# d3sm0/gym_pomdp

Hardware: AMD Instinct MI355X
Metric: env steps/sec (whole node), RockSample(7,8) batch=2^20, 1/2/4/8 MI355X (higher is better)
Workload: dtype int32

## Files before the change

### gym_pomdp_amd/csrc/episodes.hip

```cpp
#include "kernels_common.hip.h"
#include <cstring>

namespace pomdp {

template <class Env>
__global__ __launch_bounds__(BLOCK) void reset_where_kernel(const typename Env::Params p, uint32_t *__restrict__ state,
                                                            int32_t *__restrict__ ob, uint8_t *__restrict__ done,
                                                            const uint8_t *__restrict__ where, int64_t n, RngKey key, uint32_t lane0)
{
    __shared__ typename Env::Shared sh;
    Env::stage(sh, p, (int)threadIdx.x);
    __syncthreads();
    const int64_t i = (int64_t)blockIdx.x * BLOCK + threadIdx.x;
    if (i >= n) return;
    const bool fresh = !where || where[i] != 0;
    int o = -1;
    if (fresh) {
        typename Env::State st;
        o = Env::reset(sh, p, st, key, lane0 + (uint32_t)i);
        Env::store(st, state, n, (uint32_t)i, true);
        if (done) done[i] = 0;
    }
    if (ob) ob[i] = o;
}
// ... 153 lines not shown
        if constexpr (TAPE) a_tape = col.nxt;
    }
    if (in_range) {
        Env::store(st, state_w, n, rel, false);
        done[wg0 + rel] = frozen ? 1 : 0;
        if constexpr (RETS) out.finish(0, rel);
    }
    if (TAPE && n_bad && tape.err) atomicAdd(tape.err, n_bad);
}

template <class Env, class L, class Pol>
__global__ __launch_bounds__(BLOCK) void episodes_quad_kernel(uint32_t *__restrict__ state, uint8_t *__restrict__ done,
                                                              void *__restrict__ out0, void *__restrict__ out1, uint64_t discount_bits,
                                                              int64_t n, RngKey key0, uint32_t lane0, int k_steps, int64_t rec,
                                                              const typename Env::Params p, TapeRef tape)
{
    constexpr bool RETS = L::ID == LAYOUT_RETURNS;
    constexpr int W = Env::WORDS;
    using S = typename Env::S;
    __shared__ typename Env::Shared sh;
    __shared__ typename Env::RecTab tab;
    const uint32_t n_act = (uint32_t)Env::n_actions(p);
    const uint32_t l0 = blockIdx.x * (uint32_t)(4 * BLOCK) + 4u * threadIdx.x, glane0 = lane0 + l0;
    Pol pol(tape, l0, glane0, key0, key0, n_act, k_steps);
    using Out = typename std::conditional<RETS, EpisodeReturns<Env, 4>, QuadOut<L>>::type;
    Out out = [&]() {
        if constexpr (RETS) return Out(reinterpret_cast<double *>(out0), reinterpret_cast<uint32_t *>(out1), bits_f64(discount_bits), rec);
        else return Out(out0, nullptr, nullptr, nullptr, rec, l0);
    }();
    typename Env::State st[4];
    bool frozen[4];
    uint32_t a_cur[4] = {0, 0, 0, 0};
    {
        const u32x4 lo = ld_stream4(state + l0);
        u32x4 hi = {0, 0, 0, 0};
        if (W == 2) hi = ld_stream4(state + n + l0);
        const uint32_t dn = ld_stream(reinterpret_cast<const uint32_t *>(done + l0));
        if constexpr (Pol::TAPE) {
            const u32x4 f = pol.first();
#pragma unroll
            for (int j = 0; j < 4; ++j) a_cur[j] = f[j];
        }
#pragma unroll
        for (int j = 0; j < 4; ++j) {
            st[j].s = (S)((uint64_t)lo[j] | ((uint64_t)hi[j] << 32));
            frozen[j] = ((dn >> (8 * j)) & 0xFFu) != 0u;
        }
// ... 197 lines not shown
```

### gym_pomdp_amd/csrc/fused_impl.hip.h

```cpp
#pragma once
#include "kernels_common.hip.h"

namespace pomdp {

template <class L, class Pol, int LPT = 4, bool SROW = false>
struct FusedCtx {
    uint32_t l0, glane0;
    uint64_t t0;
    typename lanes_out<L, LPT, SROW>::type out;
    typename lanes_policy<Pol, LPT>::type pol;
    uint32_t n_bad;
    __device__ __forceinline__ FusedCtx(int32_t *action, int32_t *ob, void *reward, uint8_t *done, int64_t rec, uint32_t lane0,
                                        const RngKey &key0, const RngKey &akey0, uint32_t n_act, int k_steps, const TapeRef &tape)
        : l0(blockIdx.x * (uint32_t)(LPT * BLOCK) + (uint32_t)LPT * threadIdx.x), glane0(lane0 + l0),
          t0(((uint64_t)key0.t_hi << 32) | key0.t_lo), out(action, ob, reward, done, rec, l0),
          pol(tape, l0, glane0, key0, akey0, n_act, k_steps), n_bad(0) {}
    __device__ __forceinline__ void first(int gen_first, int (&a_cur)[LPT])
    {
        if constexpr (LPT == 4) {
            const u32x4 a4 = out.first(pol, gen_first);
#pragma unroll
            for (int j = 0; j < 4; ++j) a_cur[j] = (int)a4[j];
        } else {
            uint32_t a2[LPT];
            pol.first(a2);
#pragma unroll
            for (int j = 0; j < LPT; ++j) a_cur[j] = (int)a2[j];
        }
    }
    __device__ __forceinline__ RngKey key(const RngKey &key0, int s) const
    {
        RngKey k = key0;
        k.t_lo = (uint32_t)(t0 + (uint64_t)s); k.t_hi = (uint32_t)((t0 + (uint64_t)s) >> 32);
        return k;
    }
    __device__ __forceinline__ void advance(int s, uint32_t (&a_next)[LPT], int (&a_cur)[LPT])
    {
        pol.end(s, a_next);
#pragma unroll
        for (int j = 0; j < LPT; ++j) a_cur[j] = (int)a_next[j];
    }
    __device__ __forceinline__ void finish(int k_steps)
    {
        pol.count_bad(n_bad);
        out.finish(k_steps);
    }
};
#define POMDP_FUSED_STEP_LOOP(prio_, s_)                                                                              \
    wait_loads();                                                                                                      \
    _Pragma("unroll 1") for (int seg_ = 0, s_ = 0; seg_ < 4; ++seg_)                                                   \
        for (const int seg_end_ = (prio_).segment(seg_); s_ < seg_end_; ++s_)


template <class Env, int LPT, bool SIMPLE, bool TAB = false, class L = Columns, bool TAPE = false>
__global__ __launch_bounds__(BLOCK) void steps_kernel(uint32_t *__restrict__ state, int32_t *__restrict__ action,
                                                      int32_t *__restrict__ ob, typename Env::Reward *__restrict__ reward,
                                                      uint8_t *__restrict__ done, uint32_t *__restrict__ err, int64_t n,
                                                      RngKey key0, uint32_t lane0, int flags, RngKey akey0, int k_steps,
                                                      int64_t rec, const typename Env::Params p, TapeRef tape)
{
    static_assert(!TAPE || LPT == 1, "a tape drives the one-lane-per-thread instantiations");
    __shared__ typename Env::Shared sh;
    constexpr bool REC = TAB;
    __shared__ typename step_tab_of<Env, TAB>::type tab;
    static_assert(!TAB || (SIMPLE && LPT == 1), "the table-driven step serves the SIMPLE one-lane-per-thread instantiation");
    const bool auto_reset = SIMPLE || (flags & POMDP_AUTO_RESET);
    const uint32_t wg0 = blockIdx.x * (uint32_t)(BLOCK * LPT);
    const uint32_t last = SIMPLE ? (uint32_t)(BLOCK * LPT - 1) : (uint32_t)((uint64_t)(n - 1) - wg0);
    LaneOut<L, typename Env::Reward, LPT> out(action, ob, reward, done, rec, wg0);
    uint32_t *const state_w = state + wg0;
    constexpr bool COLS = L::ID == POMDP_LAYOUT_COLUMNS;
    uint32_t rel[LPT], glane[LPT];
    bool in_range[LPT], was_done[LPT], ever_fresh[LPT];
    int a_cur[LPT];
// ... 197 lines not shown
        for (int seg = 0, s = 0; seg < 4; ++seg)
        for (const int seg_end = prio.segment(seg); s < seg_end; ++s) step_body(s, s & 3);
    }
#pragma unroll
    for (int j = 0; j < LPT; ++j)
        if (in_range[j]) { Env::store(st[j], state_w, n, rel[j], ever_fresh[j]); out.finish(j, rel[j], k_steps); }
}

template <class Env, class L, class Pol, int LPT, class Form>
__device__ __forceinline__ void steps_quad_body(uint32_t *__restrict__ state, int32_t *__restrict__ action,
                                                int32_t *__restrict__ ob, int32_t *__restrict__ reward,
                                                uint8_t *__restrict__ done, int64_t n, RngKey key0, uint32_t lane0,
                                                RngKey akey0, int k_steps, int64_t rec, int gen_first,
                                                const typename Env::Params &p, TapeRef tape)
{
    static_assert(LPT == 4 || LPT == 2, "a quad or half a quad per thread");
    constexpr int W = Env::WORDS;
    using S = typename Env::S;
    __shared__ typename Env::Shared sh;
    __shared__ typename Form::Tab tab;
    const uint32_t n_act = (uint32_t)Env::n_actions(p);
    constexpr bool AHEAD2 = Pol::TAPE && LPT == 4;
    using PolT = typename std::conditional<AHEAD2, TapeQuadAhead, Pol>::type;
    FusedCtx<L, PolT, LPT, true> cx(action, ob, reward, done, rec, lane0, key0, akey0, n_act, k_steps, tape);
    const uint32_t l0 = cx.l0, glane0 = cx.glane0;
    const uint32_t e0 = LPT == 4 ? 0u : (glane0 & 2u);
    typename Env::State st[LPT];
    int a_cur[LPT];
    uint32_t sp0 = 0, sp1 = 0, gp0 = 0, gp1 = 0;
    {
        uint32_t s_lo[LPT], s_hi[LPT];
        if constexpr (LPT == 4) {
            const u32x4 lo = ld_stream4(state + l0);
            u32x4 hi = {0, 0, 0, 0};
            if (W == 2) hi = ld_stream4(state + n + l0);
#pragma unroll
            for (int j = 0; j < 4; ++j) { s_lo[j] = lo[j]; s_hi[j] = hi[j]; }
        } else {
            const u32x2 lo = ld_stream2(state + l0);
            u32x2 hi = {0, 0};
            if (W == 2) hi = ld_stream2(state + n + l0);
#pragma unroll
            for (int j = 0; j < 2; ++j) { s_lo[j] = lo[j]; s_hi[j] = hi[j]; }
        }
        cx.first(gen_first, a_cur);
#pragma unroll
        for (int j = 0; j < LPT; ++j) {
            if constexpr (W == 1) st[j].s = Form::from_mem(s_lo[j]);
            else st[j].s = (S)((uint64_t)s_lo[j] | ((uint64_t)s_hi[j] << 32));
        }
    }
    Env::stage(sh, p, (int)threadIdx.x);
    __syncthreads();
    if constexpr (W == 1) { if (Form::builds(threadIdx.x)) Form::build(tab, sh, p, (int)threadIdx.x); }
    else Env::build_rec_tab(tab, sh, p, (int)threadIdx.x);
    __syncthreads();
    const int K = p.num_rocks;
    const uint32_t start = (uint32_t)p.start_x | ((uint32_t)p.start_y << 4);
    uint32_t start_rot = start, tie_bound = 0;
    if constexpr (W == 1) { start_rot = Form::start_word(start); asm volatile("" : "+v"(start_rot)); }
    const LoopPrio prio(k_steps);
    constexpr uint32_t SENSOR_BLOCK = Env::SENSOR_BLOCK;
    const PhiloxFixed sensor_fx = philox_fixed(glane0 >> 2, ((uint32_t)POMDP_STREAM_STEP << 24) | SENSOR_BLOCK, key0.k1);
    const PhiloxFixed gate_fx = philox_fixed(glane0 >> 2, (uint32_t)POMDP_STREAM_STEP << 24, key0.k1);
    if constexpr (W == 1) tie_bound = Form::tie_bound(K);
    auto step_body = [&](const int s, const auto par_) __attribute__((always_inline)) {
        constexpr int PAR = decltype(par_)::value;
        const RngKey key = cx.key(key0, s);
        uint32_t H[LPT], G[LPT];
        if constexpr (LPT == 4) {
            const uint4 sw = philox4x32_10_fixed(sensor_fx, key.t_lo, key.t_hi, key.k0, key.k1);
            H[0] = sw.x; H[1] = sw.y; H[2] = sw.z; H[3] = sw.w;
        } else {
            pair_shared(s, e0 != 0u, [&](int sb) { return Env::quad_block(cx.key(key0, sb), glane0, SENSOR_BLOCK); }, H, sp0, sp1);
        }
        uint32_t a_next[LPT];
        if constexpr (AHEAD2) cx.pol.template begin_par<PAR>(s, a_next);
        else cx.pol.begin(s, a_next);
        bool acts[LPT];
#pragma unroll
        for (int j = 0; j < LPT; ++j) acts[j] = true;
        if constexpr (Env::STOCHASTIC) {
            if constexpr (LPT == 4) {
                const uint4 gw = philox4x32_10_fixed(gate_fx, key.t_lo, key.t_hi, key.k0, key.k1);
                G[0] = gw.x; G[1] = gw.y; G[2] = gw.z; G[3] = gw.w;
            } else {
                pair_shared(s, e0 != 0u, [&](int sb) { return Env::quad_block(cx.key(key0, sb), glane0, 0u); }, G, gp0, gp1);
            }
#pragma unroll
            for (int j = 0; j < LPT; ++j)
                acts[j] = Env::k53_le(G[j], (uint32_t)(p.act_thr >> 26), (uint32_t)p.act_thr & Env::LO_MASK,
                                      [&]() { return Env::elem(Env::quad_block(key, glane0, 1u), e0 + (uint32_t)j); }) != (p.act_gt != 0);
        }
        uint32_t rec[LPT], a_taken[LPT];
#pragma unroll
        for (int j = 0; j < LPT; ++j) a_taken[j] = (uint32_t)a_cur[j];
        bool valid[LPT];
#pragma unroll
        for (int j = 0; j < LPT; ++j) valid[j] = !Pol::TAPE || a_taken[j] < n_act;
        auto low_word = [&](int j) __attribute__((always_inline)) {
            return Env::elem(Env::quad_block(rare_key(key), glane0 + (uint32_t)j, SENSOR_BLOCK + 1u), e0 + (uint32_t)j);
        };
        if constexpr (W == 1) {
            uint32_t fresh[LPT], sn[LPT];
            typename Form::Entry ef[LPT];
            Form::template fresh<LPT>(H, key, glane0, K, start_rot, tie_bound, fresh);
#pragma unroll
// ... 43 lines not shown
                              [&]() { return low_word(j); });
                if constexpr (Env::STOCHASTIC) {
                    sj = acts[j] ? sj : st[j].s;
                    rec[j] = acts[j] ? rec[j] : a_taken[j];
                }
                if constexpr (Pol::TAPE) {
                    sj = valid[j] ? sj : st[j].s;
                    rec[j] = valid[j] ? rec[j] : a_taken[j];
                    cx.n_bad += (uint32_t)!valid[j];
                }
                st[j].s = sj;
            }
        }
        cx.out.put_records(rec, a_next);
        if constexpr (AHEAD2) {
            cx.pol.template end_par<PAR>(s, a_next);
#pragma unroll
            for (int j = 0; j < LPT; ++j) a_cur[j] = (int)a_next[j];
        } else cx.advance(s, a_next, a_cur);
    };
    if constexpr (AHEAD2) {
        wait_loads();
        _Pragma("unroll 1") for (int seg = 0, s = 0; seg < 4; ++seg)
            for (const int seg_end = prio.template segment<2>(seg); s < seg_end; s += 2) {
                step_body(s, std::integral_constant<int, 0>{});
                if (s + 1 < seg_end) step_body(s + 1, std::integral_constant<int, 1>{});
            }
    } else {
        POMDP_FUSED_STEP_LOOP(prio, s) step_body(s, std::integral_constant<int, 0>{});
    }
    cx.finish(k_steps);
    uint32_t w_lo[LPT];
#pragma unroll
    for (int j = 0; j < LPT; ++j) {
        w_lo[j] = (uint32_t)st[j].s;
        if constexpr (W == 1) w_lo[j] = Form::to_mem(w_lo[j]);
    }
    if constexpr (LPT == 4) {
        st_stream4(state + l0, w_lo[0], w_lo[1], w_lo[2], w_lo[3]);
        if (W == 2)
            st_stream4(state + n + l0, (uint32_t)((uint64_t)st[0].s >> 32), (uint32_t)((uint64_t)st[1].s >> 32),
                       (uint32_t)((uint64_t)st[2].s >> 32), (uint32_t)((uint64_t)st[3].s >> 32));
    } else {
        st_stream2(state + l0, w_lo[0], w_lo[1]);
        if (W == 2) st_stream2(state + n + l0, (uint32_t)((uint64_t)st[0].s >> 32), (uint32_t)((uint64_t)st[1].s >> 32));
    }
}
template <class Env, class L = Columns, class Pol = SyntheticQuad, int LPT = 4>
__global__ __launch_bounds__(BLOCK) void steps_quad_kernel(uint32_t *__restrict__ state, int32_t *__restrict__ action,
                                                           int32_t *__restrict__ ob, int32_t *__restrict__ reward,
                                                           uint8_t *__restrict__ done, int64_t n, RngKey key0, uint32_t lane0,
                                                           RngKey akey0, int k_steps, int64_t rec, int gen_first,
// ... 5 lines not shown
template <class Env, class L = Columns, class Pol = SyntheticQuad, int LPT = 4>
__global__ __launch_bounds__(BLOCK) void steps_quad_popc_kernel(uint32_t *__restrict__ state, int32_t *__restrict__ action,
                                                                int32_t *__restrict__ ob, int32_t *__restrict__ reward,
                                                                uint8_t *__restrict__ done, int64_t n, RngKey key0, uint32_t lane0,
                                                                RngKey akey0, int k_steps, int64_t rec, int gen_first,
                                                                const typename Env::Params p, TapeRef tape)
{
    static_assert(Env::WORDS == 1, "two state words take steps_quad_kernel");
    steps_quad_body<Env, L, Pol, LPT, typename Env::RecRot>(state, action, ob, reward, done, n, key0, lane0, akey0, k_steps, rec, gen_first, p, tape);
}

template <bool TAB, class L = Columns, class Pol = SyntheticQuad, int LPT = 4>
__global__ __launch_bounds__(BLOCK) void tag_steps_quad_kernel(uint32_t *__restrict__ state, int32_t *__restrict__ action,
                                                               int32_t *__restrict__ ob, float *__restrict__ reward,
                                                               uint8_t *__restrict__ done, int64_t n, RngKey key0,
                                                               uint32_t lane0, RngKey akey0, int k_steps, int64_t rec,
                                                               int gen_first, const TagEnv::Params p, TapeRef tape)
{
    using Env = TagEnv;
    static_assert(LPT == 4 || LPT == 2, "a quad or half a quad per thread");
    __shared__ Env::Shared sh;
    __shared__ typename std::conditional<TAB, Env::StepTab, NoTab>::type tab;
    const uint32_t n_act = (uint32_t)Env::n_actions(p);
    FusedCtx<L, Pol, LPT> cx(action, ob, reward, done, rec, lane0, key0, akey0, n_act, k_steps, tape);
    const uint32_t l0 = cx.l0, glane0 = cx.glane0;
    const uint32_t e0 = LPT == 4 ? 0u : (glane0 & 2u);
    Env::State st[LPT];
    int a_cur[LPT];
    uint32_t sp0 = 0, sp1 = 0;
    {
        if constexpr (LPT == 4) {
            const u32x4 s4 = ld_stream4(state + l0);
            cx.first(gen_first, a_cur);
#pragma unroll
            for (int j = 0; j < 4; ++j) st[j].w = s4[j];
        } else {
            const u32x2 s2 = ld_stream2(state + l0);
            cx.first(gen_first, a_cur);
#pragma unroll
            for (int j = 0; j < 2; ++j) st[j].w = s2[j];
        }
    }
    Env::stage(sh, p, (int)threadIdx.x);
    __syncthreads();
    if constexpr (TAB) {
        Env::build_tab(tab, sh, p, (int)threadIdx.x);
        __syncthreads();
    }
    const LoopPrio prio(k_steps);
    POMDP_FUSED_STEP_LOOP(prio, s) {
        const RngKey key = cx.key(key0, s);
        uint32_t a_next[LPT];
        cx.pol.begin(s, a_next);
        int o[LPT], d[LPT];
        float r[LPT];
        uint32_t a_taken[LPT], W[LPT];
#pragma unroll
        for (int j = 0; j < LPT; ++j) a_taken[j] = (uint32_t)a_cur[j];
        if constexpr (LPT == 4) {
            const uint4 qw = Env::quad_block(key, glane0, 0u);
            W[0] = qw.x; W[1] = qw.y; W[2] = qw.z; W[3] = qw.w;
        } else {
            pair_shared(s, e0 != 0u, [&](int sb) { return Env::quad_block(cx.key(key0, sb), glane0, 0u); }, W, sp0, sp1);
        }
#pragma unroll
        for (int j = 0; j < LPT; ++j) {
            Env::Flight f;
            const bool valid = !Pol::TAPE || a_taken[j] < n_act;
            const Env::State before = st[j];
            const int a = valid ? a_cur[j] : 0;
            if constexpr (TAB) Env::step_one_opponent_tab(tab, st[j], a, o[j], r[j], d[j], f);
            else Env::step_one_opponent_pre(sh, p, st[j], a, o[j], r[j], d[j], f);
            const uint32_t lane = glane0 + (uint32_t)j;
// ... 70 lines not shown
        if (threadIdx.x < 4) {
            const uint32_t f = (T.fail >> 16) - 1u, nb = (T.nb >> 16) - 1u;
            tp[threadIdx.x] = (((threadIdx.x & 1u) ? nb : f) << 16) | ((threadIdx.x & 2u) ? nb : f);
        }
    } else {
#pragma unroll
    for (int kb = 0; kb < NB; ++kb) {
        uint32_t m = 0;
        for (int i = 0; i < p.n_machines; ++i) m |= (((p.nb_mask[i] >> (8 * kb)) & threadIdx.x) != 0u ? 1u : 0u) << i;
        nbf8[kb][threadIdx.x] = m;
    }
    }
    if (threadIdx.x < 3 * 68) {
        const int kind = (int)threadIdx.x / 68, b = (int)threadIdx.x % 68;
        double r = (double)b;
        if (kind == 1) r -= .1;
        if (kind == 2) r -= 2.5;
        rtab[kind][b] = (float)r;
    }
    __syncthreads();
    const uint32_t all_up = p.n_machines >= 32 ? 0xFFFFFFFFu : ((1u << p.n_machines) - 1u);
    const int M2 = 2 * p.n_machines;
    const LoopPrio prio(k_steps);
    POMDP_FUSED_STEP_LOOP(prio, s) {
        const RngKey key = cx.key(key0, s);
        uint32_t a_next[4];
        cx.pol.begin(s, a_next);
        const uint4 q0 = Env::quad_block(key, glane0, 0u), q1 = Env::quad_block(key, glane0, 1u), q2 = Env::quad_block(key, glane0, 2u);
        const uint32_t W0[4] = {q0.x, q0.y, q0.z, q0.w}, W1[4] = {q1.x, q1.y, q1.z, q1.w};
        const uint32_t W2[4] = {q2.x, q2.y, q2.z, q2.w};
        bool valid[4] = {true, true, true, true};
        if constexpr (Pol::TAPE) {
#pragma unroll
            for (int j = 0; j < 4; ++j) { valid[j] = (uint32_t)a_cur[j] < n_act; cx.n_bad += (uint32_t)!valid[j]; }
        }
        const uint32_t a_taken[4] = {(uint32_t)a_cur[0], (uint32_t)a_cur[1], (uint32_t)a_cur[2], (uint32_t)a_cur[3]};
        if constexpr (Pol::TAPE) {
#pragma unroll
            for (int j = 0; j < 4; ++j) a_cur[j] = valid[j] ? a_cur[j] : M2;
        }
        uint32_t kill[4], todo[4], near[4], tie16[4];
        int base[4];
        bool truthful[4], pend[4], need[4];
        bool any_need = false;
#pragma unroll
        for (int j = 0; j < 4; ++j) {
            const uint32_t s0 = st[j] & all_up;
// ... 100 lines not shown
    cx.finish(k_steps);
    st_stream4(state + l0, st[0], st[1], st[2], st[3]);
}

template <class L, int MW, bool VIS_LDS = false> struct quad_waves { static constexpr int value = (L::ID == LAYOUT_RETURNS && MW >= 3 && !VIS_LDS) ? 4 : 1; };
template <int MW, class L = Columns, class Pol = SyntheticQuad, int LPT = 4, bool VIS_LDS = false>
__global__ __launch_bounds__(BLOCK) __attribute__((amdgpu_waves_per_eu(quad_waves<L, MW, VIS_LDS>::value))) void battleship_steps_quad_kernel(uint32_t *__restrict__ state, int32_t *__restrict__ action,
                                                                      int32_t *__restrict__ ob, int32_t *__restrict__ reward,
                                                                      uint8_t *__restrict__ done, int64_t n, RngKey key0,
                                                                      uint32_t lane0, RngKey akey0, int k_steps, int64_t rec,
                                                                      int gen_first, const pomdp_battleship_params p, TapeRef tape)
{
    using Env = BattleShipEnv<MW>;
    using Mask = typename Env::Mask;
    static_assert(LPT == 4 || LPT == 2, "a quad or half a quad per thread");
    constexpr int LOG = LPT == 4 ? 2 : 1;
    __shared__ uint32_t occ_lds[MW][LPT][BLOCK], next_lds[MW][LPT][BLOCK], vis_lds[VIS_LDS ? MW : 1][VIS_LDS ? LPT : 1][VIS_LDS ? BLOCK : 1];
    __shared__ uint8_t task_lds[BLOCK / 64][64 * LPT];
    __shared__ uint8_t ts_lds[BLOCK / 64][64 * LPT];
    __shared__ typename Env::SeqTables seq;
    Env::stage_seq(seq, p, (int)threadIdx.x);
    const int wv = (int)(threadIdx.x >> 6), me = (int)(threadIdx.x & 63u), tid = (int)threadIdx.x;
    const uint32_t n_act = (uint32_t)Env::n_actions(p);
    FusedCtx<L, Pol, LPT> cx(action, ob, reward, done, rec, lane0, key0, akey0, n_act, k_steps, tape);
    const uint32_t l0 = cx.l0, glane0 = cx.glane0, wave0 = glane0 - (uint32_t)LPT * (uint32_t)me;
    int rem[LPT];
    Mask vis[VIS_LDS ? 1 : LPT];
    int a_cur[LPT];
    {
        typename std::conditional<LPT == 4, u32x4, u32x2>::type w[3 * MW];
#pragma unroll
        for (int q = 0; q < 3 * MW; ++q) {
            if constexpr (LPT == 4) w[q] = ld_stream4(state + (int64_t)q * n + l0);
            else w[q] = ld_stream2(state + (int64_t)q * n + l0);
        }
        cx.first(gen_first, a_cur);
#pragma unroll
        for (int j = 0; j < LPT; ++j) {
            rem[j] = (int)(w[2 * MW - 1][j] >> 26);
            if constexpr (!VIS_LDS) vis[j].lo = vis[j].hi = 0;
#pragma unroll
            for (int q = 0; q < MW; ++q) {
                occ_lds[q][j][tid] = w[q][j];
                if constexpr (VIS_LDS) vis_lds[q][j][tid] = q == MW - 1 ? (w[MW + q][j] & 0x03FFFFFFu) : w[MW + q][j];
                else vis[j].set_word(q, w[MW + q][j]);
                next_lds[q][j][tid] = w[2 * MW + q][j];
            }
// ... 31 lines not shown
        bld.idle();
        take(my);
        while (__any(my >= 0)) {
            const uint4 b4 = philox4x32_10(wave0 + (uint32_t)bidx, bt_lo, bt_hi, ((uint32_t)POMDP_STREAM_NEXT << 24) | (blk & 0xFFFFFFu), key0.k0, key0.k1);
            ++blk;
            Env::feed2(bld, seq, bc, b4.x, b4.y);
            Env::feed2(bld, seq, bc, b4.z, b4.w);
            const bool fin = my >= 0 && !bld.busy();
            const uint64_t fm = __ballot(fin);
            if (fm != 0ull) {
                if (fin) {
#pragma unroll
                    for (int w = 0; w < MW; ++w) next_lds[w][bidx & (LPT - 1)][64 * wv + (bidx >> LOG)] = (uint32_t)(bld.occ >> (32 * w));
                }
                const int r = (int)__builtin_amdgcn_mbcnt_hi((uint32_t)(fm >> 32), __builtin_amdgcn_mbcnt_lo((uint32_t)fm, 0u));
                if (fin) { my = next_task + r < ntask ? next_task + r : -1; bld.idle(); take(my); }
                next_task += __popcll(fm);
            }
        }
        __builtin_amdgcn_fence(__ATOMIC_RELEASE, "wavefront");
        __builtin_amdgcn_wave_barrier();
    };
    const LoopPrio prio(k_steps, k_steps >= 32);
    POMDP_FUSED_STEP_LOOP(prio, s) {
        uint32_t a_taken[LPT];
        bool valid[LPT];
#pragma unroll
        for (int j = 0; j < LPT; ++j) { a_taken[j] = (uint32_t)a_cur[j]; valid[j] = true; }
        if constexpr (Pol::TAPE) {
#pragma unroll
            for (int j = 0; j < LPT; ++j) { valid[j] = a_taken[j] < n_act; cx.n_bad += (uint32_t)!valid[j]; a_cur[j] = valid[j] ? a_cur[j] : 0; }
        }
        uint32_t ow[LPT], vw[LPT];
#pragma unroll
        for (int j = 0; j < LPT; ++j) {
            ow[j] = occ_lds[a_cur[j] >> 5][j][tid];
            vw[j] = VIS_LDS ? vis_lds[a_cur[j] >> 5][j][tid] : 0u;
        }
        uint32_t a_next[LPT];
        cx.pol.begin(s, a_next);
        uint32_t o4[LPT], r4[LPT], d4[LPT];
        bool d[LPT], again = false, any_d = false;
#pragma unroll
        for (int j = 0; j < LPT; ++j) {
            const int a = a_cur[j];
            int r;
            uint32_t ob_j;
// ... 78 lines not shown
template <class Env, class L = Columns, class Pol = SyntheticQuad>
__global__ __launch_bounds__(BLOCK) void steps_quad_generic_kernel(uint32_t *__restrict__ state, int32_t *__restrict__ action,
                                                                   int32_t *__restrict__ ob,
                                                                   typename Env::Reward *__restrict__ reward,
                                                                   uint8_t *__restrict__ done, int64_t n, RngKey key0,
                                                                   uint32_t lane0, RngKey akey0, int k_steps, int64_t rec,
                                                                   int gen_first, const typename Env::Params p, TapeRef tape)
{
    static_assert(Env::WORDS == 1 && sizeof(typename Env::Reward) == 4, "one state word, 4-byte rewards");
    __shared__ typename Env::Shared sh;
    const uint32_t n_act = (uint32_t)Env::n_actions(p);
    FusedCtx<L, Pol> cx(action, ob, reward, done, rec, lane0, key0, akey0, n_act, k_steps, tape);
    const uint32_t l0 = cx.l0, glane0 = cx.glane0;
    typename Env::State st[4];
    int a_cur[4];
    {
#pragma unroll
        for (int j = 0; j < 4; ++j) Env::load(st[j], state, n, l0 + (uint32_t)j);
        cx.first(gen_first, a_cur);
    }
    Env::stage(sh, p, (int)threadIdx.x);
    __syncthreads();
    const LoopPrio prio(k_steps);
    POMDP_FUSED_STEP_LOOP(prio, s) {
        const RngKey key = cx.key(key0, s);
        uint32_t a_next[4];
        cx.pol.begin(s, a_next);
        uint32_t o4[4], r4[4], d4[4], rc[4] = {0, 0, 0, 0};
        const uint32_t a_taken[4] = {(uint32_t)a_cur[0], (uint32_t)a_cur[1], (uint32_t)a_cur[2], (uint32_t)a_cur[3]};
        uint32_t W[4] = {0, 0, 0, 0};
        if constexpr (quad_word_env<Env>::value) {
            const uint4 qw = Env::quad_block(key, glane0, 0u);
            W[0] = qw.x; W[1] = qw.y; W[2] = qw.z; W[3] = qw.w;
        }
#pragma unroll
        for (int j = 0; j < 4; ++j) {
            int o, d;
            typename Env::Reward r;
            const uint32_t lane = glane0 + (uint32_t)j;
            const bool valid = !Pol::TAPE || a_taken[j] < n_act;
            const typename Env::State before = st[j];
            const int a = valid ? a_cur[j] : 0;
            if constexpr (quad_word_env<Env>::value)
                Env::step_word(p, st[j], a, W[j], [&]() { return Env::elem(Env::quad_block(key, lane, 1u), (uint32_t)j); }, o, r, d);
            else
                Env::step(sh, p, st[j], a, key, lane, o, r, d);
            if constexpr (Pol::TAPE) { if (!valid) { st[j] = before; o = 0; r = 0; d = 0; cx.n_bad++; } }
// ... 248 lines not shown
```

### gym_pomdp_amd/csrc/philox.hip.h

```cpp
#pragma once
#include <hip/hip_runtime.h>
#include <stdint.h>

namespace pomdp {

template <bool STREAM = true, class T>
__device__ __forceinline__ T ld_stream(const T *p) { return STREAM ? __builtin_nontemporal_load(p) : *p; }
template <bool STREAM = true, class T>
__device__ __forceinline__ void st_stream(T *p, T v)
{
    if (STREAM) __hip_atomic_store(p, v, __ATOMIC_RELAXED, __HIP_MEMORY_SCOPE_AGENT);
    else *p = v;
}

typedef uint32_t u32x4 __attribute__((ext_vector_type(4)));
__device__ __forceinline__ u32x4 ld_stream4(const uint32_t *p) { return __builtin_nontemporal_load(reinterpret_cast<const u32x4 *>(p)); }
__device__ __forceinline__ void st_stream4(uint32_t *p, uint32_t a, uint32_t b, uint32_t c, uint32_t d)
{
    __builtin_nontemporal_store(u32x4{a, b, c, d}, reinterpret_cast<u32x4 *>(p));
}

typedef uint32_t u32x2 __attribute__((ext_vector_type(2)));
__device__ __forceinline__ u32x2 ld_stream2(const uint32_t *p) { return __builtin_nontemporal_load(reinterpret_cast<const u32x2 *>(p)); }
__device__ __forceinline__ void st_stream2(uint32_t *p, uint32_t a, uint32_t b)
// ... 8 lines not shown

__device__ __forceinline__ uint4 philox4x32_10(uint32_t c0, uint32_t c1, uint32_t c2, uint32_t c3,
                                               uint32_t k0, uint32_t k1)
{
#pragma unroll
    for (int r = 0; r < 10; ++r) {
        const uint64_t p0 = (uint64_t)0xD2511F53u * c0;
        const uint64_t p1 = (uint64_t)0xCD9E8D57u * c2;
        const uint32_t n0 = __builtin_amdgcn_bitop3_b32((uint32_t)(p1 >> 32), c1, k0, 0x96);
        const uint32_t n2 = __builtin_amdgcn_bitop3_b32((uint32_t)(p0 >> 32), c3, k1, 0x96);
        c1 = (uint32_t)p1;
        c3 = (uint32_t)p0;
        c0 = n0;
        c2 = n2;
        k0 += 0x9E3779B9u;
        k1 += 0xBB67AE85u;
    }
    return make_uint4(c0, c1, c2, c3);
}

struct PhiloxFixed {
    uint32_t a_lo;
    uint32_t d_hi, d_lo;
};
__device__ __forceinline__ PhiloxFixed philox_fixed(uint32_t c0, uint32_t c3, uint32_t k1)
{
    const uint64_t a = (uint64_t)0xD2511F53u * c0;
    const uint64_t d = (uint64_t)0xCD9E8D57u * ((uint32_t)(a >> 32) ^ c3 ^ k1);
    return PhiloxFixed{(uint32_t)a, (uint32_t)(d >> 32), (uint32_t)d};
}
__device__ __forceinline__ uint4 philox4x32_10_fixed(const PhiloxFixed &f, uint32_t c1, uint32_t c2, uint32_t k0, uint32_t k1)
{
    const uint64_t b = (uint64_t)0xCD9E8D57u * c2;
    const uint32_t u0 = (uint32_t)(b >> 32) ^ c1 ^ k0;
    const uint64_t c = (uint64_t)0xD2511F53u * u0;
    k0 += 0x9E3779B9u; k1 += 0xBB67AE85u;
    uint32_t x0 = f.d_hi ^ ((uint32_t)b ^ k0);
    uint32_t x2 = f.a_lo ^ ((uint32_t)(c >> 32) ^ k1);
    uint32_t x1 = f.d_lo, x3 = (uint32_t)c;
    k0 += 0x9E3779B9u; k1 += 0xBB67AE85u;
    {
        const uint64_t p0 = (uint64_t)0xD2511F53u * x0;
        const uint64_t p1 = (uint64_t)0xCD9E8D57u * x2;
        const uint32_t n0 = __builtin_amdgcn_bitop3_b32((uint32_t)(p1 >> 32), x1, k0, 0x96);
        const uint32_t n2 = (uint32_t)(p0 >> 32) ^ (x3 ^ k1);
        x1 = (uint32_t)p1; x3 = (uint32_t)p0; x0 = n0; x2 = n2;
        k0 += 0x9E3779B9u; k1 += 0xBB67AE85u;
    }
#pragma unroll
    for (int r = 3; r < 10; ++r) {
        const uint64_t p0 = (uint64_t)0xD2511F53u * x0;
        const uint64_t p1 = (uint64_t)0xCD9E8D57u * x2;
        const uint32_t n0 = __builtin_amdgcn_bitop3_b32((uint32_t)(p1 >> 32), x1, k0, 0x96);
        const uint32_t n2 = __builtin_amdgcn_bitop3_b32((uint32_t)(p0 >> 32), x3, k1, 0x96);
        x1 = (uint32_t)p1; x3 = (uint32_t)p0; x0 = n0; x2 = n2;
        k0 += 0x9E3779B9u; k1 += 0xBB67AE85u;
    }
    return make_uint4(x0, x1, x2, x3);
}

__device__ __forceinline__ RngKey rare_key(const RngKey &k)
{
    RngKey r = k;
    asm volatile("" : "+s"(r.t_lo), "+s"(r.t_hi));
    return r;
}

__device__ __forceinline__ uint4 stream_block(const RngKey &k, uint32_t lane, uint32_t stream, uint32_t block)
{
// ... 42 lines not shown
```

### gym_pomdp_amd/csrc/traj_out.hip.h

```cpp
#pragma once
#include "envs.hip.h"

namespace pomdp {

constexpr int LAYOUT_RETURNS = 100;
template <bool ACT> struct ColumnsT { static constexpr int ID = POMDP_LAYOUT_COLUMNS; static constexpr const char *NAME = "Columns"; static constexpr bool CODES = false; };
using Columns = ColumnsT<true>;
using ColumnsNoAct = ColumnsT<false>;
struct Blocked { static constexpr int ID = POMDP_LAYOUT_BLOCKED; static constexpr const char *NAME = "Blocked"; static constexpr bool CODES = false; };
struct Packed  { static constexpr int ID = POMDP_LAYOUT_PACKED;  static constexpr const char *NAME = "Packed";  static constexpr bool CODES = true; };
struct Narrow  { static constexpr int ID = POMDP_LAYOUT_NARROW;  static constexpr const char *NAME = "Narrow";  static constexpr bool CODES = true; };
template <class Env> struct Returns { static constexpr int ID = LAYOUT_RETURNS; static constexpr const char *NAME = "Returns"; static constexpr bool CODES = true; using E = Env; };

constexpr int TRAJ_BLOCK_LANES = 256;
constexpr int TRAJ_BLOCK_BYTES = 13 * TRAJ_BLOCK_LANES;

static __device__ __forceinline__ uint32_t pack_record(uint32_t a, uint32_t o, uint32_t rcode, uint32_t d)
{
    return a | (o << 8) | ((rcode & 0xFFu) << 16) | (d << 24);
}

struct TapeRef {
    const uint8_t *base;
    int64_t stride;
// ... 1 lines not shown
};

template <class T>
struct TapeColumn {
    const uint8_t *p;
    int64_t stride;
    int last;
    T first, nxt;
    __device__ __forceinline__ T row(int r) const
    {
        r = r < last ? r : last;
        return ld_stream(reinterpret_cast<const T *>(p + (int64_t)r * stride));
    }
    __device__ __forceinline__ TapeColumn(const TapeRef &t, uint32_t col, int k_steps)
        : p(t.base + col), stride(t.stride), last(k_steps - 1), nxt(0) { first = row(0); }
    __device__ __forceinline__ void request(int s) { nxt = row(s + 1); }
};
struct NoColumn {
    uint8_t first, nxt;
    __device__ __forceinline__ NoColumn(const TapeRef &, uint32_t, int) : first(0), nxt(0) {}
    __device__ __forceinline__ void request(int) {}
};

struct SyntheticQuad {
    static constexpr bool TAPE = false;
    uint32_t glane0, n_act, k0, k1;
    uint64_t ta0;
    PhiloxFixed fx;
    __device__ __forceinline__ SyntheticQuad(const TapeRef &, uint32_t, uint32_t glane0_, const RngKey &key0, const RngKey &akey0, uint32_t n_act_, int)
        : glane0(glane0_), n_act(n_act_), k0(key0.k0), k1(key0.k1), ta0(((uint64_t)akey0.t_hi << 32) | akey0.t_lo),
          fx(philox_fixed(glane0_ >> 2, (uint32_t)POMDP_STREAM_ACTION << 24, key0.k1)) {}
    __device__ __forceinline__ uint4 block(uint64_t ta) const
    {
        return philox4x32_10_fixed(fx, (uint32_t)ta, (uint32_t)(ta >> 32), k0, k1);
    }
    __device__ __forceinline__ u32x4 first() const
    {
        const uint4 w = block(ta0 - 1ull);
        return u32x4{__umulhi(w.x, n_act), __umulhi(w.y, n_act), __umulhi(w.z, n_act), __umulhi(w.w, n_act)};
    }
    __device__ __forceinline__ void begin(int s, uint32_t (&a)[4]) const
    {
        const uint4 pw = block(ta0 + (uint64_t)s);
        a[0] = __umulhi(pw.x, n_act); a[1] = __umulhi(pw.y, n_act); a[2] = __umulhi(pw.z, n_act); a[3] = __umulhi(pw.w, n_act);
    }
    __device__ __forceinline__ void end(int, uint32_t (&)[4]) const {}
    __device__ __forceinline__ void count_bad(uint32_t) const {}
};
struct TapeQuad {
    static constexpr bool TAPE = true;
    TapeColumn<uint32_t> col;
    uint32_t *err;
    static __device__ __forceinline__ void unpack(uint32_t w, uint32_t (&a)[4])
    {
        a[0] = w & 0xFFu; a[1] = __builtin_amdgcn_ubfe(w, 8u, 8u); a[2] = __builtin_amdgcn_ubfe(w, 16u, 8u); a[3] = w >> 24;
    }
    __device__ __forceinline__ TapeQuad(const TapeRef &t, uint32_t l0, uint32_t, const RngKey &, const RngKey &, uint32_t, int k_steps)
        : col(t, l0, k_steps), err(t.err) {}
    __device__ __forceinline__ u32x4 first() const
    {
        uint32_t a[4];
        unpack(col.first, a);
        return u32x4{a[0], a[1], a[2], a[3]};
    }
    __device__ __forceinline__ void begin(int s, uint32_t (&a)[4]) { col.request(s); a[0] = a[1] = a[2] = a[3] = 0; }
    __device__ __forceinline__ void end(int, uint32_t (&a)[4]) const { unpack(col.nxt, a); }
    __device__ __forceinline__ void count_bad(uint32_t n_bad) const { if (n_bad && err) atomicAdd(err, n_bad); }
};

struct TapeQuadAhead {
    static constexpr bool TAPE = true;
    TapeColumn<uint32_t> col;
    uint32_t *err;
    uint32_t even, odd;
    __device__ __forceinline__ TapeQuadAhead(const TapeRef &t, uint32_t l0, uint32_t, const RngKey &, const RngKey &, uint32_t, int k_steps)
        : col(t, l0, k_steps), err(t.err), even(0), odd(col.row(1)) {}
    __device__ __forceinline__ u32x4 first() const
    {
        uint32_t a[4];
        TapeQuad::unpack(col.first, a);
        return u32x4{a[0], a[1], a[2], a[3]};
    }
    template <int PAR> __device__ __forceinline__ void begin_par(int s, uint32_t (&a)[4])
    {
        if constexpr (PAR == 0) even = col.row(s + 2); else odd = col.row(s + 2);
        a[0] = a[1] = a[2] = a[3] = 0;
    }
    template <int PAR> __device__ __forceinline__ void end_par(int, uint32_t (&a)[4]) const { TapeQuad::unpack(PAR == 0 ? odd : even, a); }
    __device__ __forceinline__ void count_bad(uint32_t n_bad) const { if (n_bad && err) atomicAdd(err, n_bad); }
};

static __device__ __forceinline__ uint32_t pair_swap(uint32_t v)
{
    return (uint32_t)__builtin_amdgcn_update_dpp((int)v, (int)v, 0xB1, 0xF, 0xF, false);
}
template <class BlockOfStep>
static __device__ __forceinline__ void pair_shared(int s, bool hi, BlockOfStep block_of_step, uint32_t (&w)[2], uint32_t &odd0, uint32_t &odd1)
{
    if ((s & 1) == 0) {
        const uint4 b = block_of_step(s + (hi ? 1 : 0));
        const uint32_t r0 = pair_swap(hi ? b.x : b.z), r1 = pair_swap(hi ? b.y : b.w);
        w[0] = hi ? r0 : b.x; w[1] = hi ? r1 : b.y;
        odd0 = hi ? b.z : r0; odd1 = hi ? b.w : r1;
    } else { w[0] = odd0; w[1] = odd1; }
}
struct SyntheticPair {
    static constexpr bool TAPE = false;
    uint32_t glane0, n_act, k0, k1, odd[2];
    uint64_t ta0;
    bool hi;
    __device__ __forceinline__ SyntheticPair(const TapeRef &, uint32_t, uint32_t glane0_, const RngKey &key0, const RngKey &akey0, uint32_t n_act_, int)
        : glane0(glane0_), n_act(n_act_), k0(key0.k0), k1(key0.k1), odd{0, 0}, ta0(((uint64_t)akey0.t_hi << 32) | akey0.t_lo), hi((glane0_ & 2u) != 0u) {}
    __device__ __forceinline__ uint4 block(uint64_t ta) const
    {
        return philox4x32_10(glane0 >> 2, (uint32_t)ta, (uint32_t)(ta >> 32), (uint32_t)POMDP_STREAM_ACTION << 24, k0, k1);
    }
    __device__ __forceinline__ void first(uint32_t (&a)[2]) const
    {
        const uint4 w = block(ta0 - 1ull);
        a[0] = __umulhi(hi ? w.z : w.x, n_act); a[1] = __umulhi(hi ? w.w : w.y, n_act);
    }
    __device__ __forceinline__ void begin(int s, uint32_t (&a)[2])
    {
        if ((s & 1) == 0) {
            const uint4 w = block(ta0 + (uint64_t)s + (hi ? 1ull : 0ull));
            const uint32_t r0 = pair_swap(hi ? w.x : w.z), r1 = pair_swap(hi ? w.y : w.w);
            a[0] = __umulhi(hi ? r0 : w.x, n_act); a[1] = __umulhi(hi ? r1 : w.y, n_act);
            odd[0] = __umulhi(hi ? w.z : r0, n_act); odd[1] = __umulhi(hi ? w.w : r1, n_act);
        } else { a[0] = odd[0]; a[1] = odd[1]; }
    }
    __device__ __forceinline__ void end(int, uint32_t (&)[2]) const {}
    __device__ __forceinline__ void count_bad(uint32_t) const {}
};
struct TapePair {
    static constexpr bool TAPE = true;
    TapeColumn<uint16_t> col;
    uint32_t *err;
    __device__ __forceinline__ TapePair(const TapeRef &t, uint32_t l0, uint32_t, const RngKey &, const RngKey &, uint32_t, int k_steps)
        : col(t, l0, k_steps), err(t.err) {}
    __device__ __forceinline__ void first(uint32_t (&a)[2]) const { a[0] = col.first & 0xFFu; a[1] = (uint32_t)col.first >> 8; }
    __device__ __forceinline__ void begin(int s, uint32_t (&a)[2]) { col.request(s); a[0] = a[1] = 0; }
    __device__ __forceinline__ void end(int, uint32_t (&a)[2]) const { a[0] = col.nxt & 0xFFu; a[1] = (uint32_t)col.nxt >> 8; }
    __device__ __forceinline__ void count_bad(uint32_t n_bad) const { if (n_bad && err) atomicAdd(err, n_bad); }
};
template <class Pol, int LPT> struct lanes_policy { using type = Pol; };
template <> struct lanes_policy<SyntheticQuad, 2> { using type = SyntheticPair; };
template <> struct lanes_policy<TapeQuad, 2> { using type = TapePair; };

template <class L> struct QuadOut;

template <bool ACT> struct QuadOut<ColumnsT<ACT>> {
    uint32_t *action_w, *ob_w, *reward_w, *done_w;
    int64_t rec;
    __device__ __forceinline__ QuadOut(void *action, void *ob, void *reward, void *done, int64_t rec_, uint32_t l0)
        : action_w(ACT ? reinterpret_cast<uint32_t *>(action) + l0 : nullptr), ob_w(reinterpret_cast<uint32_t *>(ob) + l0),
          reward_w(reinterpret_cast<uint32_t *>(reward) + l0), done_w(reinterpret_cast<uint32_t *>(reinterpret_cast<uint8_t *>(done) + l0)),
          rec(rec_) {}
    template <class Pol>
    __device__ __forceinline__ u32x4 first(const Pol &pol, int gen_first)
    {
        if constexpr (!ACT) return pol.first();
        u32x4 a;
        if (!gen_first) a = ld_stream4(action_w);
        else {
            a = pol.first();
            st_stream4(action_w, a[0], a[1], a[2], a[3]);
        }
        action_w += rec;
        return a;
    }
// ... 480 lines not shown
```

Baseline: 1022 billion.

## Hoist step-invariant Philox first-round multiply out of the step loop into stretches

```diff
diff --git a/gym_pomdp_amd/csrc/episodes.hip b/gym_pomdp_amd/csrc/episodes.hip
--- a/gym_pomdp_amd/csrc/episodes.hip
+++ b/gym_pomdp_amd/csrc/episodes.hip
@@ -199,7 +199,7 @@
     __shared__ typename Env::RecTab tab;
     const uint32_t n_act = (uint32_t)Env::n_actions(p);
     const uint32_t l0 = blockIdx.x * (uint32_t)(4 * BLOCK) + 4u * threadIdx.x, glane0 = lane0 + l0;
-    Pol pol(tape, l0, glane0, key0, key0, n_act, k_steps);
+    typename lanes_policy<Pol, 4, false>::type pol(tape, l0, glane0, key0, key0, n_act, k_steps);
     using Out = typename std::conditional<RETS, EpisodeReturns<Env, 4>, QuadOut<L>>::type;
     Out out = [&]() {
         if constexpr (RETS) return Out(reinterpret_cast<double *>(out0), reinterpret_cast<uint32_t *>(out1), bits_f64(discount_bits), rec);
diff --git a/gym_pomdp_amd/csrc/fused_impl.hip.h b/gym_pomdp_amd/csrc/fused_impl.hip.h
--- a/gym_pomdp_amd/csrc/fused_impl.hip.h
+++ b/gym_pomdp_amd/csrc/fused_impl.hip.h
@@ -3,12 +3,13 @@
 
 namespace pomdp {
 
-template <class L, class Pol, int LPT = 4, bool SROW = false>
+template <class L, bool TIGHT> constexpr bool hoist_fits = !(TIGHT && L::ID == LAYOUT_RETURNS);
+template <class L, class Pol, int LPT = 4, bool SROW = false, bool HOIST = true>
 struct FusedCtx {
     uint32_t l0, glane0;
     uint64_t t0;
     typename lanes_out<L, LPT, SROW>::type out;
-    typename lanes_policy<Pol, LPT>::type pol;
+    typename lanes_policy<Pol, LPT, HOIST>::type pol;
     uint32_t n_bad;
     __device__ __forceinline__ FusedCtx(int32_t *action, int32_t *ob, void *reward, uint8_t *done, int64_t rec, uint32_t lane0,
                                         const RngKey &key0, const RngKey &akey0, uint32_t n_act, int k_steps, const TapeRef &tape)
@@ -28,6 +29,7 @@
             for (int j = 0; j < LPT; ++j) a_cur[j] = (int)a2[j];
         }
     }
+    __device__ __forceinline__ int stretch(int s, int end) { return pol.stretch(s, end); }
     __device__ __forceinline__ RngKey key(const RngKey &key0, int s) const
     {
         RngKey k = key0;
@@ -46,10 +48,11 @@
         out.finish(k_steps);
     }
 };
-#define POMDP_FUSED_STEP_LOOP(prio_, s_)                                                                              \
+#define POMDP_FUSED_STEP_LOOP(prio_, s_, stretch_)                                                                    \
     wait_loads();                                                                                                      \
     _Pragma("unroll 1") for (int seg_ = 0, s_ = 0; seg_ < 4; ++seg_)                                                   \
-        for (const int seg_end_ = (prio_).segment(seg_); s_ < seg_end_; ++s_)
+        _Pragma("unroll 1") for (const int seg_end_ = (prio_).segment(seg_); s_ < seg_end_;)                           \
+            _Pragma("unroll 1") for (const int end_ = stretch_(s_, seg_end_); s_ < end_; ++s_)
 
 
 template <class Env, int LPT, bool SIMPLE, bool TAB = false, class L = Columns, bool TAPE = false>
@@ -293,7 +296,8 @@
     const uint32_t n_act = (uint32_t)Env::n_actions(p);
     constexpr bool AHEAD2 = Pol::TAPE && LPT == 4;
     using PolT = typename std::conditional<AHEAD2, TapeQuadAhead, Pol>::type;
-    FusedCtx<L, PolT, LPT, true> cx(action, ob, reward, done, rec, lane0, key0, akey0, n_act, k_steps, tape);
+    constexpr bool HOIST = hoist_fits<L, Env::STOCHASTIC>;
+    FusedCtx<L, PolT, LPT, true, HOIST> cx(action, ob, reward, done, rec, lane0, key0, akey0, n_act, k_steps, tape);
     const uint32_t l0 = cx.l0, glane0 = cx.glane0;
     const uint32_t e0 = LPT == 4 ? 0u : (glane0 & 2u);
     typename Env::State st[LPT];
@@ -332,15 +336,33 @@
     if constexpr (W == 1) { start_rot = Form::start_word(start); asm volatile("" : "+v"(start_rot)); }
     const LoopPrio prio(k_steps);
     constexpr uint32_t SENSOR_BLOCK = Env::SENSOR_BLOCK;
-    const PhiloxFixed sensor_fx = philox_fixed(glane0 >> 2, ((uint32_t)POMDP_STREAM_STEP << 24) | SENSOR_BLOCK, key0.k1);
-    const PhiloxFixed gate_fx = philox_fixed(glane0 >> 2, (uint32_t)POMDP_STREAM_STEP << 24, key0.k1);
+    constexpr int NFX = AHEAD2 ? 2 : 1;
+    PhiloxFixed sensor_fx[NFX], gate_fx[NFX];
+#pragma unroll
+    for (int h = 0; h < NFX; ++h) {
+        sensor_fx[h] = philox_fixed(glane0 >> 2, ((uint32_t)POMDP_STREAM_STEP << 24) | SENSOR_BLOCK, key0.k1);
+        gate_fx[h] = philox_fixed(glane0 >> 2, (uint32_t)POMDP_STREAM_STEP << 24, key0.k1);
+    }
+    auto stretch = [&](const int s, int end) __attribute__((always_inline)) {
+        end = cx.stretch(s, end);
+        if constexpr (LPT == 4 && HOIST) {
+#pragma unroll
+            for (int h = 0; h < NFX; ++h) {
+                const RngKey kh = cx.key(key0, s + h);
+                philox_hoist(sensor_fx[h], kh.t_hi, kh.k0);
+                if constexpr (Env::STOCHASTIC) philox_hoist(gate_fx[h], kh.t_hi, kh.k0);
+                end = stretch_end<NFX>(s, end, kh.t_lo);
+            }
+        }
+        return end;
+    };
     if constexpr (W == 1) tie_bound = Form::tie_bound(K);
     auto step_body = [&](const int s, const auto par_) __attribute__((always_inline)) {
         constexpr int PAR = decltype(par_)::value;
         const RngKey key = cx.key(key0, s);
         uint32_t H[LPT], G[LPT];
         if constexpr (LPT == 4) {
-            const uint4 sw = philox4x32_10_fixed(sensor_fx, key.t_lo, key.t_hi, key.k0, key.k1);
+            const uint4 sw = philox4x32_10_fixed<HOIST>(sensor_fx[AHEAD2 ? PAR : 0], key.t_lo, key.t_hi, key.k0, key.k1);
             H[0] = sw.x; H[1] = sw.y; H[2] = sw.z; H[3] = sw.w;
         } else {
             pair_shared(s, e0 != 0u, [&](int sb) { return Env::quad_block(cx.key(key0, sb), glane0, SENSOR_BLOCK); }, H, sp0, sp1);
@@ -353,7 +375,7 @@
         for (int j = 0; j < LPT; ++j) acts[j] = true;
         if constexpr (Env::STOCHASTIC) {
             if constexpr (LPT == 4) {
-                const uint4 gw = philox4x32_10_fixed(gate_fx, key.t_lo, key.t_hi, key.k0, key.k1);
+                const uint4 gw = philox4x32_10_fixed<HOIST>(gate_fx[AHEAD2 ? PAR : 0], key.t_lo, key.t_hi, key.k0, key.k1);
                 G[0] = gw.x; G[1] = gw.y; G[2] = gw.z; G[3] = gw.w;
             } else {
                 pair_shared(s, e0 != 0u, [&](int sb) { return Env::quad_block(cx.key(key0, sb), glane0, 0u); }, G, gp0, gp1);
@@ -443,12 +465,13 @@
     if constexpr (AHEAD2) {
         wait_loads();
         _Pragma("unroll 1") for (int seg = 0, s = 0; seg < 4; ++seg)
-            for (const int seg_end = prio.template segment<2>(seg); s < seg_end; s += 2) {
-                step_body(s, std::integral_constant<int, 0>{});
-                if (s + 1 < seg_end) step_body(s + 1, std::integral_constant<int, 1>{});
-            }
+            _Pragma("unroll 1") for (const int seg_end = prio.template segment<2>(seg); s < seg_end;)
+                _Pragma("unroll 1") for (const int end = stretch(s, seg_end); s < end; s += 2) {
+                    step_body(s, std::integral_constant<int, 0>{});
+                    if (s + 1 < end) step_body(s + 1, std::integral_constant<int, 1>{});
+                }
     } else {
-        POMDP_FUSED_STEP_LOOP(prio, s) step_body(s, std::integral_constant<int, 0>{});
+        POMDP_FUSED_STEP_LOOP(prio, s, stretch) step_body(s, std::integral_constant<int, 0>{});
     }
     cx.finish(k_steps);
     uint32_t w_lo[LPT];
@@ -500,7 +523,7 @@
     __shared__ Env::Shared sh;
     __shared__ typename std::conditional<TAB, Env::StepTab, NoTab>::type tab;
     const uint32_t n_act = (uint32_t)Env::n_actions(p);
-    FusedCtx<L, Pol, LPT> cx(action, ob, reward, done, rec, lane0, key0, akey0, n_act, k_steps, tape);
+    FusedCtx<L, Pol, LPT, false, L::ID != POMDP_LAYOUT_NARROW> cx(action, ob, reward, done, rec, lane0, key0, akey0, n_act, k_steps, tape);
     const uint32_t l0 = cx.l0, glane0 = cx.glane0;
     const uint32_t e0 = LPT == 4 ? 0u : (glane0 & 2u);
     Env::State st[LPT];
@@ -526,7 +549,7 @@
         __syncthreads();
     }
     const LoopPrio prio(k_steps);
-    POMDP_FUSED_STEP_LOOP(prio, s) {
+    POMDP_FUSED_STEP_LOOP(prio, s, cx.stretch) {
         const RngKey key = cx.key(key0, s);
         uint32_t a_next[LPT];
         cx.pol.begin(s, a_next);
@@ -643,7 +666,7 @@
     const uint32_t all_up = p.n_machines >= 32 ? 0xFFFFFFFFu : ((1u << p.n_machines) - 1u);
     const int M2 = 2 * p.n_machines;
     const LoopPrio prio(k_steps);
-    POMDP_FUSED_STEP_LOOP(prio, s) {
+    POMDP_FUSED_STEP_LOOP(prio, s, cx.stretch) {
         const RngKey key = cx.key(key0, s);
         uint32_t a_next[4];
         cx.pol.begin(s, a_next);
@@ -790,7 +813,7 @@
     Env::stage_seq(seq, p, (int)threadIdx.x);
     const int wv = (int)(threadIdx.x >> 6), me = (int)(threadIdx.x & 63u), tid = (int)threadIdx.x;
     const uint32_t n_act = (uint32_t)Env::n_actions(p);
-    FusedCtx<L, Pol, LPT> cx(action, ob, reward, done, rec, lane0, key0, akey0, n_act, k_steps, tape);
+    FusedCtx<L, Pol, LPT, false, hoist_fits<L, true>> cx(action, ob, reward, done, rec, lane0, key0, akey0, n_act, k_steps, tape);
     const uint32_t l0 = cx.l0, glane0 = cx.glane0, wave0 = glane0 - (uint32_t)LPT * (uint32_t)me;
     int rem[LPT];
     Mask vis[VIS_LDS ? 1 : LPT];
@@ -868,7 +891,7 @@
         __builtin_amdgcn_wave_barrier();
     };
     const LoopPrio prio(k_steps, k_steps >= 32);
-    POMDP_FUSED_STEP_LOOP(prio, s) {
+    POMDP_FUSED_STEP_LOOP(prio, s, cx.stretch) {
         uint32_t a_taken[LPT];
         bool valid[LPT];
 #pragma unroll
@@ -993,7 +1016,7 @@
     Env::stage(sh, p, (int)threadIdx.x);
     __syncthreads();
     const LoopPrio prio(k_steps);
-    POMDP_FUSED_STEP_LOOP(prio, s) {
+    POMDP_FUSED_STEP_LOOP(prio, s, cx.stretch) {
         const RngKey key = cx.key(key0, s);
         uint32_t a_next[4];
         cx.pol.begin(s, a_next);
diff --git a/gym_pomdp_amd/csrc/philox.hip.h b/gym_pomdp_amd/csrc/philox.hip.h
--- a/gym_pomdp_amd/csrc/philox.hip.h
+++ b/gym_pomdp_amd/csrc/philox.hip.h
@@ -54,29 +54,46 @@
 struct PhiloxFixed {
     uint32_t a_lo;
     uint32_t d_hi, d_lo;
+    uint32_t q_hi, q_lo;
 };
 __device__ __forceinline__ PhiloxFixed philox_fixed(uint32_t c0, uint32_t c3, uint32_t k1)
 {
     const uint64_t a = (uint64_t)0xD2511F53u * c0;
     const uint64_t d = (uint64_t)0xCD9E8D57u * ((uint32_t)(a >> 32) ^ c3 ^ k1);
-    return PhiloxFixed{(uint32_t)a, (uint32_t)(d >> 32), (uint32_t)d};
+    return PhiloxFixed{(uint32_t)a, (uint32_t)(d >> 32), (uint32_t)d, 0u, 0u};
 }
-__device__ __forceinline__ uint4 philox4x32_10_fixed(const PhiloxFixed &f, uint32_t c1, uint32_t c2, uint32_t k0, uint32_t k1)
+__device__ __forceinline__ void philox_hoist(PhiloxFixed &f, uint32_t c2, uint32_t k0)
 {
+    const uint32_t x0 = f.d_hi ^ ((0xCD9E8D57u * c2) ^ (k0 + 0x9E3779B9u));
+    const uint64_t q = (uint64_t)0xD2511F53u * x0;
+    f.q_hi = (uint32_t)(q >> 32); f.q_lo = (uint32_t)q;
+}
+template <int UNIT = 1>
+__device__ __forceinline__ int stretch_end(int s, int end, uint32_t t_lo)
+{
+    uint32_t more = 0u - t_lo - 1u;
+    if (UNIT == 2) more |= 1u;
+    const uint32_t room = (uint32_t)(end - s - 1);
+    return s + 1 + (int)(room < more ? room : more);
+}
+template <bool HOIST = true>
+__device__ __forceinline__ uint4 philox4x32_10_fixed(const PhiloxFixed &fixed, uint32_t c1, uint32_t c2, uint32_t k0, uint32_t k1)
+{
+    PhiloxFixed f = fixed;
+    if (!HOIST) philox_hoist(f, c2, k0);
     const uint64_t b = (uint64_t)0xCD9E8D57u * c2;
     const uint32_t u0 = (uint32_t)(b >> 32) ^ c1 ^ k0;
     const uint64_t c = (uint64_t)0xD2511F53u * u0;
     k0 += 0x9E3779B9u; k1 += 0xBB67AE85u;
-    uint32_t x0 = f.d_hi ^ ((uint32_t)b ^ k0);
+    uint32_t x0;
     uint32_t x2 = f.a_lo ^ ((uint32_t)(c >> 32) ^ k1);
     uint32_t x1 = f.d_lo, x3 = (uint32_t)c;
     k0 += 0x9E3779B9u; k1 += 0xBB67AE85u;
     {
-        const uint64_t p0 = (uint64_t)0xD2511F53u * x0;
         const uint64_t p1 = (uint64_t)0xCD9E8D57u * x2;
         const uint32_t n0 = __builtin_amdgcn_bitop3_b32((uint32_t)(p1 >> 32), x1, k0, 0x96);
-        const uint32_t n2 = (uint32_t)(p0 >> 32) ^ (x3 ^ k1);
-        x1 = (uint32_t)p1; x3 = (uint32_t)p0; x0 = n0; x2 = n2;
+        const uint32_t n2 = f.q_hi ^ (x3 ^ k1);
+        x1 = (uint32_t)p1; x3 = f.q_lo; x0 = n0; x2 = n2;
         k0 += 0x9E3779B9u; k1 += 0xBB67AE85u;
     }
 #pragma unroll
diff --git a/gym_pomdp_amd/csrc/traj_out.hip.h b/gym_pomdp_amd/csrc/traj_out.hip.h
--- a/gym_pomdp_amd/csrc/traj_out.hip.h
+++ b/gym_pomdp_amd/csrc/traj_out.hip.h
@@ -47,21 +47,30 @@
     __device__ __forceinline__ void request(int) {}
 };
 
-struct SyntheticQuad {
+template <bool HOIST>
+struct SyntheticQuadT {
     static constexpr bool TAPE = false;
     uint32_t glane0, n_act, k0, k1;
     uint64_t ta0;
     PhiloxFixed fx;
-    __device__ __forceinline__ SyntheticQuad(const TapeRef &, uint32_t, uint32_t glane0_, const RngKey &key0, const RngKey &akey0, uint32_t n_act_, int)
+    __device__ __forceinline__ SyntheticQuadT(const TapeRef &, uint32_t, uint32_t glane0_, const RngKey &key0, const RngKey &akey0, uint32_t n_act_, int)
         : glane0(glane0_), n_act(n_act_), k0(key0.k0), k1(key0.k1), ta0(((uint64_t)akey0.t_hi << 32) | akey0.t_lo),
           fx(philox_fixed(glane0_ >> 2, (uint32_t)POMDP_STREAM_ACTION << 24, key0.k1)) {}
+    __device__ __forceinline__ int stretch(int s, int end)
+    {
+        if constexpr (!HOIST) return end;
+        const uint64_t ta = ta0 + (uint64_t)s;
+        philox_hoist(fx, (uint32_t)(ta >> 32), k0);
+        return stretch_end(s, end, (uint32_t)ta);
+    }
     __device__ __forceinline__ uint4 block(uint64_t ta) const
     {
-        return philox4x32_10_fixed(fx, (uint32_t)ta, (uint32_t)(ta >> 32), k0, k1);
+        return philox4x32_10_fixed<HOIST>(fx, (uint32_t)ta, (uint32_t)(ta >> 32), k0, k1);
     }
     __device__ __forceinline__ u32x4 first() const
     {
-        const uint4 w = block(ta0 - 1ull);
+        const uint64_t ta = ta0 - 1ull;
+        const uint4 w = philox4x32_10_fixed<false>(fx, (uint32_t)ta, (uint32_t)(ta >> 32), k0, k1);
         return u32x4{__umulhi(w.x, n_act), __umulhi(w.y, n_act), __umulhi(w.z, n_act), __umulhi(w.w, n_act)};
     }
     __device__ __forceinline__ void begin(int s, uint32_t (&a)[4]) const
@@ -72,6 +81,8 @@
     __device__ __forceinline__ void end(int, uint32_t (&)[4]) const {}
     __device__ __forceinline__ void count_bad(uint32_t) const {}
 };
+struct SyntheticQuad : SyntheticQuadT<true> { using SyntheticQuadT<true>::SyntheticQuadT; };
+struct SyntheticQuadPlain : SyntheticQuadT<false> { using SyntheticQuadT<false>::SyntheticQuadT; };
 struct TapeQuad {
     static constexpr bool TAPE = true;
     TapeColumn<uint32_t> col;
@@ -91,6 +102,7 @@
     __device__ __forceinline__ void begin(int s, uint32_t (&a)[4]) { col.request(s); a[0] = a[1] = a[2] = a[3] = 0; }
     __device__ __forceinline__ void end(int, uint32_t (&a)[4]) const { unpack(col.nxt, a); }
     __device__ __forceinline__ void count_bad(uint32_t n_bad) const { if (n_bad && err) atomicAdd(err, n_bad); }
+    __device__ __forceinline__ int stretch(int, int end) const { return end; }
 };
 
 struct TapeQuadAhead {
@@ -113,6 +125,7 @@
     }
     template <int PAR> __device__ __forceinline__ void end_par(int, uint32_t (&a)[4]) const { TapeQuad::unpack(PAR == 0 ? odd : even, a); }
     __device__ __forceinline__ void count_bad(uint32_t n_bad) const { if (n_bad && err) atomicAdd(err, n_bad); }
+    __device__ __forceinline__ int stretch(int, int end) const { return end; }
 };
 
 static __device__ __forceinline__ uint32_t pair_swap(uint32_t v)
@@ -156,6 +169,7 @@
     }
     __device__ __forceinline__ void end(int, uint32_t (&)[2]) const {}
     __device__ __forceinline__ void count_bad(uint32_t) const {}
+    __device__ __forceinline__ int stretch(int, int end) const { return end; }
 };
 struct TapePair {
     static constexpr bool TAPE = true;
@@ -167,10 +181,12 @@
     __device__ __forceinline__ void begin(int s, uint32_t (&a)[2]) { col.request(s); a[0] = a[1] = 0; }
     __device__ __forceinline__ void end(int, uint32_t (&a)[2]) const { a[0] = col.nxt & 0xFFu; a[1] = (uint32_t)col.nxt >> 8; }
     __device__ __forceinline__ void count_bad(uint32_t n_bad) const { if (n_bad && err) atomicAdd(err, n_bad); }
-};
-template <class Pol, int LPT> struct lanes_policy { using type = Pol; };
-template <> struct lanes_policy<SyntheticQuad, 2> { using type = SyntheticPair; };
-template <> struct lanes_policy<TapeQuad, 2> { using type = TapePair; };
+    __device__ __forceinline__ int stretch(int, int end) const { return end; }
+};
+template <class Pol, int LPT, bool HOIST = true> struct lanes_policy { using type = Pol; };
+template <bool HOIST> struct lanes_policy<SyntheticQuad, 2, HOIST> { using type = SyntheticPair; };
+template <bool HOIST> struct lanes_policy<TapeQuad, 2, HOIST> { using type = TapePair; };
+template <> struct lanes_policy<SyntheticQuad, 4, false> { using type = SyntheticQuadPlain; };
 
 template <class L> struct QuadOut;
 
```

Result: faster. 1038 billion (median of 6 runs) (+1.6%).
